# antoineleeman/robust-nonlinear-mpc

Hardware: AMD Instinct MI355X
Metric: QP solves/sec (whole node), rockETH N=20 batch=4096 closed-loop RTI MPC step from script x0 (higher is better)
Workload: dtype f64

## Files before the change

robust-nonlinear-mpc_amd/csrc/dynamics.hpp:

```cpp
#pragma once
#include <math.h>
#ifndef __HIPCC__
#ifndef __host__
#define __host__
#endif
#ifndef __device__
#define __device__
#endif
#endif
#define DYN_HD __host__ __device__ inline

namespace dyn {

struct Dual {
    double v, d;
    DYN_HD Dual() : v(0.0), d(0.0) {}
    DYN_HD Dual(double a) : v(a), d(0.0) {}
    DYN_HD Dual(double a, double b) : v(a), d(b) {}
};
DYN_HD Dual operator+(Dual a, Dual b) { return Dual(a.v + b.v, a.d + b.d); }
DYN_HD Dual operator-(Dual a, Dual b) { return Dual(a.v - b.v, a.d - b.d); }
DYN_HD Dual operator-(Dual a) { return Dual(-a.v, -a.d); }
DYN_HD Dual operator*(Dual a, Dual b) { return Dual(a.v * b.v, a.d * b.v + a.v * b.d); }
DYN_HD Dual operator/(Dual a, Dual b) { const double q = a.v / b.v; return Dual(q, (a.d - q * b.d) / b.v); }
DYN_HD Dual msin(Dual a) { return Dual(sin(a.v), cos(a.v) * a.d); }
DYN_HD Dual mcos(Dual a) { return Dual(cos(a.v), -sin(a.v) * a.d); }
DYN_HD Dual msqrt(Dual a) { const double s = sqrt(a.v); return Dual(s, 0.5 * a.d / s); }
DYN_HD Dual matan(Dual a) { return Dual(atan(a.v), a.d / (1.0 + a.v * a.v)); }
DYN_HD void msincos(double a, double &s, double &c) {
#ifdef __HIP_DEVICE_COMPILE__
    sincos(a, &s, &c);
#else
    s = sin(a); c = cos(a);
#endif
}
DYN_HD void msincos(Dual a, Dual &s, Dual &c) {
    double sv, cv;
    msincos(a.v, sv, cv);
    s = Dual(sv, cv * a.d); c = Dual(cv, -sv * a.d);
}
DYN_HD double msin(double a) { return sin(a); }
DYN_HD double mcos(double a) { return cos(a); }
DYN_HD double msqrt(double a) { return sqrt(a); }
// ... 148 lines not shown
    constexpr int NX = Dims<MODEL>::NX, NT = Dims<MODEL>::NT;
    const double h = RK4_H;
    double k[NX], t[NX], acc[NX];
    { MathRecord mf(tape); ode<MODEL, double, MathRecord>(x, u, k, mf); }
    for (int i = 0; i < NX; i++) { acc[i] = k[i]; t[i] = x[i] + 0.5 * h * k[i]; stage[i] = t[i]; }
    { MathRecord mf(tape + NT); ode<MODEL, double, MathRecord>(t, u, k, mf); }
    for (int i = 0; i < NX; i++) { acc[i] = acc[i] + 2.0 * k[i]; t[i] = x[i] + 0.5 * h * k[i]; stage[NX + i] = t[i]; }
    { MathRecord mf(tape + 2 * NT); ode<MODEL, double, MathRecord>(t, u, k, mf); }
    for (int i = 0; i < NX; i++) { acc[i] = acc[i] + 2.0 * k[i]; t[i] = x[i] + h * k[i]; stage[2 * NX + i] = t[i]; }
    { MathRecord mf(tape + 3 * NT); ode<MODEL, double, MathRecord>(t, u, k, mf); }
    for (int i = 0; i < NX; i++) xp[i] = x[i] + (1.0 / 6.0) * (acc[i] + k[i]) * h;
}
template <int MODEL>
DYN_HD void ddyn_tangent(const double *x, const double *u, const double *stage, const double *tape, int dir, double *col) {
    constexpr int NX = Dims<MODEL>::NX, NU = Dims<MODEL>::NU, NT = Dims<MODEL>::NT;
    const double h = RK4_H;
    Dual T[NX], U[NU], K[NX];
    double acc[NX];
    for (int i = 0; i < NU; i++) U[i] = Dual(u[i], NX + i == dir ? 1.0 : 0.0);
    for (int i = 0; i < NX; i++) { T[i] = Dual(x[i], i == dir ? 1.0 : 0.0); acc[i] = 0.0; }
#pragma unroll
    for (int s = 0; s < 4; s++) {
        { MathReplay mf(tape + s * NT); ode<MODEL, Dual, MathReplay>(T, U, K, mf); }
        const double w = (s == 0 || s == 3) ? 1.0 : 2.0, cn = (s == 2) ? h : 0.5 * h;
        for (int i = 0; i < NX; i++) {
            acc[i] += w * K[i].d;
            if (s < 3) T[i] = Dual(stage[s * NX + i], (i == dir ? 1.0 : 0.0) + cn * K[i].d);
        }
    }
    for (int i = 0; i < NX; i++) col[i] = (i == dir ? 1.0 : 0.0) + (h / 6.0) * acc[i];
}

}
```

robust-nonlinear-mpc_amd/csrc/slsqp_api.hip:

```cpp
#include <hip/hip_runtime.h>

#include <algorithm>
#include <cmath>
#include <cstdio>
#include <cstring>
#include <cstdlib>
#include <map>
#include <string>
#include <vector>

#include "../../include/slsqp.h"
#include "slsqp_kernels.hpp"

using namespace slsqp;

static thread_local std::string g_err;
static int fail(const std::string &m) { g_err = m; return -1; }
#define HIPCHK(x)                                                                                  \
    do {                                                                                           \
        hipError_t e_ = (x);                                                                       \
        if (e_ != hipSuccess) return fail(std::string(#x) + ": " + hipGetErrorString(e_));         \
    } while (0)

extern "C" const char *slsqp_last_error(void) { return g_err.c_str(); }
extern "C" const char *slsqp_version(void) { return "slsqp-hip 0.1 (gfx950)"; }

extern "C" void slsqp_default_opts(slsqp_opts *o) {
    o->rti_steps = 1; o->max_sls_iter = 30; o->qp_max_iter = 60; o->qp_eps = 1e-6; o->conv_tol = 1e-3;
    o->eps_backoff = 1e-10; o->want_K = 1; o->warm_start = 1; o->warm_rounds = 20;
    o->max_scp_iter = 100; o->scp_eps = 1e-10; o->precision = 0; o->time_kernels = 0; o->as_first = 2; o->as_rounds = 24; o->as_max_viol = 64; o->ipm_restart = 1; o->as_warm_max_set = 28; o->as_warm_last = 1; o->fuse_rti = 1; o->cl_persistent = 1;
}

struct slsqp_handle {
    slsqp_dims d;
    int B, dev, n, m, mb, nz;
    hipStream_t st;
    double *A, *Bm, *E, *g, *gN, *c, *q, *x0val, *gf_raw, *g_raw, *cst;
    int model_id;
    double *Xn, *Un, *xmeas, *x0arg, *u0, *wbuf, *u_init; int cl_steps;
    double *ubg, *lbg;
    double *primal, *dual, *cost, *pin_dual, *kkt, *prev_primal, *Linv, *ws, *qpstate;
    double *eta, *eta_f, *beta, *beta_f, *backoff, *backoff_f, *backoff_x, *backoff_u, *K;
    int *status, *iters, *itnum, *has_prev, *conv, *alive, *mask, *success, *infeas, *counter;
    int *scp_active, *scp_success, *scp_iters, *pending_reset, *scp_upd; double *scp_dmax;
    int horizon_shifted = 0;
    std::vector<hipEvent_t> tl; std::vector<int> tl_role; int tl_n = 0; double tl_acc[5] = {0, 0, 0, 0, 0};
    int *cl_stepno = nullptr, *cl_lag = nullptr, *cl_begin = nullptr, *cl_runm = nullptr, *cl_done = nullptr, *cl_skipb = nullptr, *cl_skip_begin = nullptr, *qplog = nullptr;
    double *call_ids = nullptr, *cl_W = nullptr; size_t cl_W_doubles = 0; unsigned long long *t0word = nullptr; int qplog_steps = 0, qplog_cap = 0, *qplog_nsolves = nullptr;
    int *clq_slots = nullptr, *clq_ctl = nullptr; unsigned clq_cap = 0; int cl_loop_waves = 0; double cl_loop_ms = 0.0; unsigned long long *cl_busy = nullptr, *cl_tbegin = nullptr, cl_busy_host[16] = {};
    bool cl_round = false; unsigned long long cl_budget = 0; int cl_total_steps = 0; unsigned cl_cut_count = 0xFFFFFFFFu;
    unsigned long long *chain_times = nullptr, *chain_times_host = nullptr;
    int *qp_diag = nullptr;
    double *nom_st; int *nom_need_lin, *nom_status, *nom_iters;
    int *retry; int mx_retry, mx_retry_total;
    int *databad, *runq;
    double *Kc, *Aclc;
    double *lin_stage, *lin_tape;
    double call_id;
    int *qpstat;
    double *x0viol;
    double x0_box_tol = 0.0;
    double x0_tol_dev = 0.0;
    double *x0vlog = nullptr;
    double *lg_x0v = nullptr;
    int *stale;
    double *pinf; double t_jac;
    int *mapA, *mapB;
    double *stage;
    size_t stage_bytes;
    bool have_costs, have_cons, have_dyn;
    bool beta_inited;
    bool general_G;
    double *Gd, *Gfd;
    hipEvent_t ev[10];
    std::vector<hipEvent_t> kev;
    int n_kev; bool time_kernels;
    double t_total, t_qp, t_sweep, t_fwd; int n_fwd; double fwd_inst;
    std::map<std::string, std::pair<void *, size_t>> named;
    unsigned long long *inst_launches;
    double *ct_part, *cost_tube;
    std::vector<void *> owned, log_owned;
    int log_steps;
    double *lg_x, *lg_u, *lg_bx, *lg_bu, *lg_state, *lg_u0, *lg_pinf; int *lg_succ, *lg_it;
};

static Costs costs_of(slsqp_handle *h) {
    const int nx = h->d.nx, nu = h->d.nu;
    Costs c;
    c.Qd = h->cst; c.Rd = c.Qd + nx; c.Qfd = c.Rd + nu; c.Qregd = c.Qfd + nx; c.Rregd = c.Qregd + nx; c.Qregfd = c.Rregd + nu; c.prox = 0.0;
    return c;
// ... 43 lines not shown
    if (d->N < 1 || d->N > 64 || batch < 1) { fail("need 1 <= N <= 64 and batch >= 1"); return nullptr; }
    int ndev = 0;
    if (hipGetDeviceCount(&ndev) != hipSuccess || ndev == 0) { fail("no HIP device visible: libslsqp_hip has no CPU fallback"); return nullptr; }
    if (hipSetDevice(device) != hipSuccess) { fail("hipSetDevice failed"); return nullptr; }
    slsqp_handle *h = new slsqp_handle();
    h->d = *d; h->B = batch; h->dev = device;
    const int nx = d->nx, nu = d->nu, N = d->N, ni = d->ni, nif = d->ni_f, nw = d->nw;
    h->nz = nx + nu; h->n = h->nz * N + nx; h->mb = N * (nx + ni) + nif; h->m = h->mb + nx;
    const size_t B = batch;
    if (hipStreamCreate(&h->st) != hipSuccess) { fail("hipStreamCreate"); delete h; return nullptr; }
    int rc = 0;
    rc |= dalloc(h->owned, &h->A, B * N * nx * nx); rc |= dalloc(h->owned, &h->Bm, B * N * nx * nu); rc |= dalloc(h->owned, &h->E, (size_t)(N + 1) * nx * nx);
    (void)nw;
    rc |= dalloc(h->owned, &h->g, B * N * ni); rc |= dalloc(h->owned, &h->gN, B * nif); rc |= dalloc(h->owned, &h->c, B * N * nx); rc |= dalloc(h->owned, &h->q, B * h->n);
    rc |= dalloc(h->owned, &h->x0val, B * nx); rc |= dalloc(h->owned, &h->gf_raw, (size_t)nif); rc |= dalloc(h->owned, &h->g_raw, (size_t)ni);
    rc |= dalloc(h->owned, &h->Xn, B * (N + 1) * nx); rc |= dalloc(h->owned, &h->Un, B * N * nu); rc |= dalloc(h->owned, &h->xmeas, B * nx); rc |= dalloc(h->owned, &h->x0arg, B * nx);
    rc |= dalloc(h->owned, &h->u0, B * nu); rc |= dalloc(h->owned, &h->wbuf, B * nx); rc |= dalloc(h->owned, &h->u_init, (size_t)nu); h->cl_steps = 0; rc |= dalloc(h->owned, &h->cst, (size_t)(3 * nx + 2 * nu) * 2);
    rc |= dalloc(h->owned, &h->ubg, B * h->mb); rc |= dalloc(h->owned, &h->lbg, B * h->mb);
    rc |= dalloc(h->owned, &h->primal, B * h->n); rc |= dalloc(h->owned, &h->dual, B * h->mb); rc |= dalloc(h->owned, &h->cost, B); rc |= dalloc(h->owned, &h->pin_dual, B * nx);
    rc |= dalloc(h->owned, &h->kkt, kkt_doubles(B)); rc |= dalloc(h->owned, &h->prev_primal, B * h->n); rc |= dalloc(h->owned, &h->Linv, B * N * nx * nx); rc |= dalloc(h->owned, &h->ws, B * qp_ws_doubles(h->n, N, nx)); rc |= dalloc(h->owned, &h->qpstate, B * 40);
    rc |= dalloc(h->owned, &h->eta, B * N * N * ni); rc |= dalloc(h->owned, &h->eta_f, B * (N + 1) * nif); rc |= dalloc(h->owned, &h->beta, B * N * N * ni);
    rc |= dalloc(h->owned, &h->beta_f, B * (N + 1) * nif); rc |= dalloc(h->owned, &h->backoff, B * N * ni); rc |= dalloc(h->owned, &h->backoff_f, B * nif);
    rc |= dalloc(h->owned, &h->backoff_x, B * (N + 1) * nx); rc |= dalloc(h->owned, &h->backoff_u, B * N * nu); rc |= dalloc(h->owned, &h->K, B * N * (N + 1) * nu * nx);
    rc |= dalloc(h->owned, &h->status, B); rc |= dalloc(h->owned, &h->iters, B); rc |= dalloc(h->owned, &h->itnum, B); rc |= dalloc(h->owned, &h->has_prev, B); rc |= dalloc(h->owned, &h->conv, B);
    rc |= dalloc(h->owned, &h->alive, B); rc |= dalloc(h->owned, &h->mask, B); rc |= dalloc(h->owned, &h->success, B); rc |= dalloc(h->owned, &h->infeas, B); rc |= dalloc(h->owned, &h->counter, (size_t)4);
    rc |= dalloc(h->owned, &h->scp_active, B); rc |= dalloc(h->owned, &h->scp_success, B); rc |= dalloc(h->owned, &h->scp_iters, B); rc |= dalloc(h->owned, &h->pending_reset, B); rc |= dalloc(h->owned, &h->scp_dmax, B);
    rc |= dalloc(h->owned, &h->retry, B); h->mx_retry = 0; h->mx_retry_total = 0; rc |= dalloc(h->owned, &h->databad, B); rc |= dalloc(h->owned, &h->runq, B);
    rc |= dalloc(h->owned, &h->nom_st, B * 12); rc |= dalloc(h->owned, &h->nom_need_lin, B); rc |= dalloc(h->owned, &h->nom_status, B); rc |= dalloc(h->owned, &h->nom_iters, B);
    rc |= dalloc(h->owned, &h->mapA, (size_t)N * nx * nx); rc |= dalloc(h->owned, &h->mapB, (size_t)N * nx * nu);
    rc |= dalloc(h->owned, &h->inst_launches, (size_t)8); rc |= dalloc(h->owned, &h->chain_times, B * 4);
    rc |= dalloc(h->owned, &h->cl_stepno, B); rc |= dalloc(h->owned, &h->cl_lag, B); rc |= dalloc(h->owned, &h->cl_begin, B); rc |= dalloc(h->owned, &h->cl_runm, B); rc |= dalloc(h->owned, &h->cl_done, B);
    { unsigned cap = 1; while (cap < 4u * (unsigned)B) cap <<= 1; h->clq_cap = cap; rc |= dalloc(h->owned, &h->clq_slots, (size_t)cap); rc |= dalloc(h->owned, &h->clq_ctl, (size_t)8); rc |= dalloc(h->owned, &h->cl_busy, (size_t)16); rc |= dalloc(h->owned, &h->cl_tbegin, (size_t)B); }
    rc |= dalloc(h->owned, &h->cl_skipb, B); rc |= dalloc(h->owned, &h->call_ids, B); rc |= dalloc(h->owned, &h->t0word, (size_t)2); rc |= dalloc(h->owned, &h->ct_part, B * (N + 1)); rc |= dalloc(h->owned, &h->cost_tube, B);
    rc |= dalloc(h->owned, &h->lin_stage, B * N * 3 * nx); rc |= dalloc(h->owned, &h->lin_tape, B * N * 4 * dyn::NT_MAX); rc |= dalloc(h->owned, &h->Kc, B * N * nu * nx); rc |= dalloc(h->owned, &h->Aclc, B * N * nx * nx); rc |= dalloc(h->owned, &h->qpstat, B * 16); rc |= dalloc(h->owned, &h->Gd, (size_t)ni * (nx + nu)); rc |= dalloc(h->owned, &h->Gfd, (size_t)nif * nx); h->general_G = false; h->beta_inited = false; rc |= dalloc(h->owned, &h->stale, B); rc |= dalloc(h->owned, &h->pinf, B); rc |= dalloc(h->owned, &h->scp_upd, B); h->t_jac = 0;
    h->log_steps = 0; h->lg_x = h->lg_u = h->lg_bx = h->lg_bu = h->lg_state = h->lg_u0 = h->lg_pinf = nullptr; h->lg_succ = h->lg_it = nullptr;
    if (rc) { free_all(h->owned); hipStreamDestroy(h->st); delete h; return nullptr; }
    if (hipHostMalloc((void **)&h->chain_times_host, 4 * sizeof(unsigned long long)) != hipSuccess) h->chain_times_host = nullptr;
    else memset(h->chain_times_host, 0, 4 * sizeof(unsigned long long));
    for (auto &e : h->ev) hipEventCreate(&e);
    h->tl.resize(2 * 256); for (auto &e : h->tl) hipEventCreate(&e);
    h->tl_role.assign(256, 0); h->tl_n = 0;
    h->kev.resize(2 * 256); for (auto &e : h->kev) hipEventCreate(&e);
    h->n_kev = 0; h->t_fwd = 0; h->n_fwd = 0; h->fwd_inst = 0; h->time_kernels = false; h->call_id = 0;
    {
        std::vector<int> mA((size_t)N * nx * nx), mB((size_t)N * nx * nu);
        int p = 0;
        for (int k = 0; k <= N; k++) {
            for (int j = 0; j < nx; j++) {
                if (k >= 1) p += 1;
                if (k < N) { for (int i = 0; i < nx; i++) mA[((size_t)k * nx + i) * nx + j] = p + i; p += nx; p += 2; }
                else p += 2;
                if (k == 0) p += 1;
            }
            if (k < N)
                for (int a = 0; a < nu; a++) {
                    for (int i = 0; i < nx; i++) mB[((size_t)k * nx + i) * nu + a] = p + i;
                    p += nx; p += 2;
                }
        }
        hipMemcpyAsync(h->mapA, mA.data(), mA.size() * sizeof(int), hipMemcpyHostToDevice, h->st);
        hipMemcpyAsync(h->mapB, mB.data(), mB.size() * sizeof(int), hipMemcpyHostToDevice, h->st);
        hipStreamSynchronize(h->st);
    }
    h->stage = nullptr; h->stage_bytes = 0;
    h->have_costs = h->have_cons = h->have_dyn = false; h->model_id = -1;
    h->t_total = h->t_qp = h->t_sweep = 0;
    auto reg = [&](const char *nm, void *p, size_t bytes) { h->named[nm] = {p, bytes}; };
// ... 432 lines not shown
    for (unsigned i = blockIdx.x * blockDim.x + threadIdx.x; i < cap; i += gridDim.x * blockDim.x) q.slots[i] = (i < (unsigned)B) ? (int)i + 1 : 0;
    if (blockIdx.x == 0 && threadIdx.x == 0) { *q.head = 0u; *q.tail = (unsigned)B; *q.avail = B; *q.err = 0; }
}
__device__ __forceinline__ void solve_begin_wave(const SolveBeginArgs &a, int b, int lane) {
    const int act = a.active ? a.active[b] : 1;
    if (a.x0 && lane < a.NX) a.x0val[(size_t)b * a.NX + lane] = -a.x0[(size_t)b * a.NX + lane];
    const int pend = a.pending[b];
    wla::wsync_mem();
    if (lane == 0) { a.alive[b] = act; a.infeas[b] = 0; a.success[b] = 0; }
    if (pend && act) {
        for (size_t o = lane; o < a.neta; o += 64) a.eta[(size_t)b * a.neta + o] = 0.0;
        for (size_t o = lane; o < a.netaf; o += 64) a.eta_f[(size_t)b * a.netaf + o] = 0.0;
        const int st = a.stale[b];
        wla::wsync_mem();
        if (lane == 0) { a.itnum[b] = 0; a.pending[b] = 0; a.stale[b] = st & ~16; }
    }
    const InitBackoffArgs &i = a.ib;
    if (i.run && !i.run[b]) return;
    const int NZ = i.NX + i.NU, NI = 2 * NZ, NIF = 2 * i.NX, N = i.N;
    const double sq = sqrt(i.eps);
    for (int o = lane; o < N * NI; o += 64) i.backoff[(size_t)b * N * NI + o] = N * sq;
    for (int o = lane; o < NIF; o += 64) i.backoff_f[(size_t)b * NIF + o] = (N + 1) * sq;
    for (int o = lane; o < (N + 1) * i.NX; o += 64) i.backoff_x[(size_t)b * (N + 1) * i.NX + o] = 0.0;
    for (int o = lane; o < N * i.NU; o += 64) i.backoff_u[(size_t)b * N * i.NU + o] = 0.0;
}
struct LoopArgs {
    ChainArgs c; ClArgs cl; LinArgs lin; BoundsArgs ba; SolveBeginArgs sb; ClLogArgs lg; ScpArgs sa;
    int steps, n, have_log, fence, keep_laggards;
    int *stepno; double *call_ids, *q; int *stale, *itnum, *pending, *scp_active;
    const double *W_all; double *pinf;
    ClQueue Q;
    unsigned long long *busy, *t_begin;
};
template <int MODEL>
__device__ CLW_FN void cl_step_begin(const LoopArgs &L, int b, int lane) {
    constexpr int NX = dyn::Dims<MODEL>::NX;
    const int s = L.stepno[b];
    if (lane == 0) L.t_begin[b] = wall_clock64();
#ifdef CL_LOOP_STAMP
    unsigned long long ts_ = wall_clock64();
#define CLSTAMP(i) do { wla::wsync_mem(); const unsigned long long t_ = wall_clock64(); if (lane == 0) atomicAdd(L.busy + (i), t_ - ts_); ts_ = t_; } while (0)
#else
#define CLSTAMP(i) do {} while (0)
#endif
    if (s > 0) {
        cl_shift_wave<MODEL>(L.cl, b, lane);
        for (int o = lane; o < L.n; o += 64) L.q[(size_t)b * L.n + o] = 0.0;
        const int st = L.stale[b];
        wla::wsync_mem();
        if (lane == 0) { L.stale[b] = (st & 8) | 3; L.itnum[b] = 0; L.pending[b] = 0; }
    }
    if (lane == 0) { L.call_ids[b] += 1.0; L.sa.scp_success[b] = 0; L.sa.scp_iters[b] = 0; }
    wla::wsync_mem();
    CLSTAMP(4);
    lin_wave<MODEL>(L.lin, L.ba, b, lane);
    CLSTAMP(5);
    if (lane < NX) L.cl.x0arg[(size_t)b * NX + lane] = L.cl.Xn[(size_t)b * (L.cl.N + 1) * NX + lane] - L.cl.xmeas[(size_t)b * NX + lane];
    wla::wsync_mem();
    solve_begin_wave(L.sb, b, lane);
    wla::wsync_mem();
    CLSTAMP(6);
}
template <int MODEL>
__device__ CLW_FN int cl_step_end(const LoopArgs &L, int b, int lane) {
    constexpr int NX = dyn::Dims<MODEL>::NX;
    const int s = L.stepno[b];
#ifdef CL_LOOP_STAMP
    unsigned long long ts_ = wall_clock64();
#endif
    if (lane == 0) L.scp_active[b] = 1;
    wla::wsync_mem();
    cl_scp_update_wave(L.cl, L.sa, b, lane);
    wla::wsync_mem();
    CLSTAMP(7);
    if (L.sa.updated[b]) cl_infeas_wave<MODEL>(L.cl, L.pinf, b, lane);
    wla::wsync_mem();
    CLSTAMP(8);
    if (L.have_log) {
        const int per = 2 * ((L.lg.N + 1) * L.lg.NX + L.lg.N * L.lg.NU);
        for (int o = lane; o < per; o += 64) cl_log_item(L.lg, b, o);
    }
    CLSTAMP(9);
    if (lane == 0) {
        cl_plant_one<MODEL>(L.cl, b, L.W_all ? L.W_all + (size_t)s * L.cl.B * NX : nullptr);
        L.stepno[b] = s + 1;
        if (L.busy) { atomicAdd(L.busy, wall_clock64() - L.t_begin[b]); atomicAdd(L.busy + 2, 1ULL); }
    }
    wla::wsync_mem();
    CLSTAMP(10);
    return (s + 1 < L.steps) ? s + 1 : 0;
}
template <int MODEL>
__global__ __launch_bounds__(64, QP_PERSIST_WAVES_PER_SIMD) void k_cl_loop(LoopArgs L) {
    constexpr int NX = dyn::Dims<MODEL>::NX, NU = dyn::Dims<MODEL>::NU;
    int lane = threadIdx.x;
    extern __shared__ double sm[];
    int b = -1;
#ifdef CL_LOOP_STAMP
    const unsigned long long tw0_ = wall_clock64();
    if (lane == 0) atomicMin(L.busy + 14, tw0_);
#endif
#pragma unroll 1
    for (;;) {
        asm volatile("" : "+v"(lane));
        if (b < 0) {
#ifdef CL_LOOP_STAMP
            const unsigned long long tp_ = wall_clock64();
#endif
            b = clq_pop(L.Q, lane);
            if (b < 0) break;
            if (L.fence & 1) __threadfence();
#ifdef CL_LOOP_STAMP
            if (lane == 0) atomicAdd(L.busy + 11, wall_clock64() - tp_);
#endif
        }
        cl_step_begin<MODEL>(L, b, lane);
        b = __builtin_amdgcn_readfirstlane(b);
        asm volatile("" : "+v"(lane));
        rti_chain_dev<NX, NU>(L.c, b, lane, sm);
        wla::wsync_mem();
        asm volatile("" : "+v"(lane));
        const int next = __builtin_amdgcn_readfirstlane(cl_step_end<MODEL>(L, b, lane));
        b = __builtin_amdgcn_readfirstlane(b);
        if (!next) { b = -1; continue; }
        const unsigned long long done_steps = __hip_atomic_load(L.busy + 2, __ATOMIC_RELAXED, __HIP_MEMORY_SCOPE_AGENT);
        const int behind = __builtin_amdgcn_readfirstlane(((unsigned long long)next * (unsigned long long)L.cl.B < done_steps) ? 1 : 0);
        if (behind && L.keep_laggards) continue;
#ifdef CL_LOOP_STAMP
        const unsigned long long tq_ = wall_clock64();
#endif
        if (L.fence & 2) __threadfence();
        clq_push(L.Q, b, lane);
        b = -1;
#ifdef CL_LOOP_STAMP
        if (lane == 0) atomicAdd(L.busy + 12, wall_clock64() - tq_);
#endif
    }
#ifdef CL_LOOP_STAMP
    if (lane == 0) { const unsigned long long te_ = wall_clock64(); atomicAdd(L.busy + 13, te_ - tw0_); atomicMax(L.busy + 15, te_); atomicAdd(L.busy + 1, 1ULL); }
#endif
}

struct ScpLoopArgs {
    LoopArgs L;
    int max_it, converge, rti_steps;
    int *nsolves;
};
template <int MODEL>
__device__ CLW_FN void cl_scp_step_begin(const LoopArgs &L, int b, int lane) {
    const int s = L.stepno[b];
    if (lane == 0) L.t_begin[b] = wall_clock64();
    if (s > 0) {
        cl_shift_wave<MODEL>(L.cl, b, lane);
        for (int o = lane; o < L.n; o += 64) L.q[(size_t)b * L.n + o] = 0.0;
        const int st = L.stale[b];
// ... 840 lines not shown
                     h->pinf, h->lg_x, h->lg_u, h->lg_bx, h->lg_bu, h->lg_state, h->lg_u0, h->lg_pinf, h->lg_succ, h->lg_it};
        hipLaunchKernelGGL(k_cl_log, dim3(1024), dim3(256), 0, h->st, la);
        hipLaunchKernelGGL(k_cl_log_x0v, dim3((2 * h->B + 255) / 256), dim3(256), 0, h->st, h->B, h->log_steps, h->cl_steps, h->x0viol, h->qpstat, h->lg_x0v);
        h->named["log_x0_viol"] = {h->lg_x0v, sizeof(double) * 2 * (size_t)h->log_steps};
    }
    if (h->model_id == 0) hipLaunchKernelGGL((k_cl_shift_plant<0>), dim3(gb), dim3(64), 0, h->st, a, 0, 1);
    else if (h->model_id == 1) hipLaunchKernelGGL((k_cl_shift_plant<1>), dim3(gb), dim3(64), 0, h->st, a, 0, 1);
    else hipLaunchKernelGGL((k_cl_shift_plant<2>), dim3(gb), dim3(64), 0, h->st, a, 0, 1);
    HIPCHK(hipGetLastError());
    HIPCHK(hipStreamSynchronize(h->st));
    tl_take(h);
    h->cl_steps++;
    return 0;
}

__global__ void k_cl_begin_flags(int B, const int *begin, int *scp_success, int *scp_iters) {
    const int b = blockIdx.x * blockDim.x + threadIdx.x;
    if (b < B && begin[b]) { scp_success[b] = 0; scp_iters[b] = 0; }
}
template <int MODEL>
static int launch_loop_t(slsqp_handle *h, LoopArgs &L, const ScpLoopArgs *S = nullptr) {
    constexpr int NX = dyn::Dims<MODEL>::NX, NU = dyn::Dims<MODEL>::NU;
    const size_t lds = sizeof(double) * std::max({(size_t)qp_lds_doubles<NX, NU>(h->d.N), (size_t)(2 * h->n + 8), (size_t)sweep_lds_doubles<NX, NU>(), (size_t)sweep_prop_lds_doubles<NX, NU>()});
    int cu = 0;
    if (hipDeviceGetAttribute(&cu, hipDeviceAttributeMultiprocessorCount, h->dev) != hipSuccess || cu <= 0) cu = 256;
    const int env_waves = getenv("SLSQP_LOOP_WAVES") ? atoi(getenv("SLSQP_LOOP_WAVES")) : 0;
    const int slots = env_waves > 0 ? env_waves : cu * 4 * QP_PERSIST_WAVES_PER_SIMD;
    const int grid = std::max(1, std::min(h->B, slots));
    h->cl_loop_waves = grid;
    const bool timed = h->time_kernels && h->n_kev + 2 <= (int)h->kev.size();
    if (timed) hipEventRecord(h->kev[h->n_kev], h->st);
    hipEventRecord(h->ev[8], h->st);
    if (S) hipLaunchKernelGGL((k_cl_loop_scp<MODEL>), dim3(grid), dim3(64), lds, h->st, *S);
    else hipLaunchKernelGGL((k_cl_loop<MODEL>), dim3(grid), dim3(64), lds, h->st, L);
    hipEventRecord(h->ev[9], h->st);
    if (timed) { hipEventRecord(h->kev[h->n_kev + 1], h->st); h->n_kev += 2; }
    HIPCHK(hipGetLastError());
    return 0;
}
static int cl_run_persistent(slsqp_handle *h, int steps, const double *dW, const slsqp_opts &o, int *rounds_out, bool scp = false, int scp_rti = 1) {
    const int max_it = !scp ? 1 : (scp_rti > 0 ? scp_rti : o.max_scp_iter);
    const slsqp_dims &d = h->d;
    const int B = h->B;
    if (!h->beta_inited) {
        hipLaunchKernelGGL(k_fill_doubles, dim3(1024), dim3(256), 0, h->st, h->beta, o.eps_backoff, (size_t)B * d.N * d.N * d.ni);
        hipLaunchKernelGGL(k_fill_doubles, dim3(1024), dim3(256), 0, h->st, h->beta_f, o.eps_backoff, (size_t)B * (d.N + 1) * d.ni_f);
        h->beta_inited = true;
    }
    h->time_kernels = o.time_kernels != 0;
    LoopArgs L;
    const int *active = scp ? h->scp_active : nullptr;
    L.c = make_chain_args(h, o, active, 1);
    L.c.q1.call_ids = L.c.q2.call_ids = h->call_ids;
    L.c.q1.shift_stepno = L.c.q2.shift_stepno = h->cl_stepno;
    L.c.qplog = h->qplog; L.c.x0vlog = h->x0vlog; L.c.stepno = h->cl_stepno; L.c.log_steps = h->qplog_steps;
    L.cl = cl_args(h, nullptr);
    L.lin = LinArgs{B, d.N, h->Xn, h->Un, h->g_raw, h->gf_raw, costs_of(h), h->A, h->Bm, h->c, h->g, h->gN, h->q, nullptr, h->lin_stage, h->lin_tape};
    L.ba = BoundsArgs{B, d.N, d.nx, d.ni, d.ni_f, h->g, h->gN, h->c, h->ubg, h->lbg, 1e-10, nullptr};
    L.sb = SolveBeginArgs{B, d.nx, h->x0arg, h->x0val, active, h->alive, h->infeas, h->success, h->pending_reset, h->itnum, h->stale,
                          h->eta, h->eta_f, (size_t)d.N * d.N * d.ni, (size_t)(d.N + 1) * d.ni_f,
                          InitBackoffArgs{B, d.N, d.nx, d.nu, o.eps_backoff, active, h->beta, h->beta_f, h->backoff, h->backoff_f, h->backoff_x, h->backoff_u, 0}, nullptr};
    L.lg = ClLogArgs{h->cl_stepno, nullptr, B, d.N, d.nx, d.nu, h->log_steps, 0, h->Xn, h->Un, h->backoff_x, h->backoff_u, h->scp_success, h->scp_iters,
                     h->pinf, h->lg_x, h->lg_u, h->lg_bx, h->lg_bu, h->lg_state, h->lg_u0, h->lg_pinf, h->lg_succ, h->lg_it};
    L.sa = ScpArgs{0, 0, o.scp_eps, h->scp_active, h->scp_success, h->scp_iters, h->counter + 2, h->scp_dmax, h->scp_upd};
    L.steps = steps; L.n = h->n; L.have_log = h->log_steps > 0 ? 1 : 0;
    L.keep_laggards = getenv("SLSQP_LOOP_KEEP") ? atoi(getenv("SLSQP_LOOP_KEEP")) : 1;
    L.fence = getenv("SLSQP_LOOP_FENCE") ? atoi(getenv("SLSQP_LOOP_FENCE")) : 3;
    L.stepno = h->cl_stepno; L.call_ids = h->call_ids; L.q = h->q; L.stale = h->stale; L.itnum = h->itnum; L.pending = h->pending_reset; L.scp_active = h->scp_active;
    L.W_all = dW; L.pinf = h->pinf;
    L.Q = ClQueue{h->clq_slots, h->clq_cap - 1u, (unsigned *)h->clq_ctl, (unsigned *)h->clq_ctl + 1, h->clq_ctl + 2, h->clq_ctl + 3};
    L.busy = h->cl_busy; L.t_begin = h->cl_tbegin;
    hipLaunchKernelGGL(k_clq_init, dim3(64), dim3(256), 0, h->st, B, L.Q);
    HIPCHK(hipMemsetAsync(h->cl_busy, 0, 16 * sizeof(unsigned long long), h->st));
    HIPCHK(hipMemsetAsync(h->cl_busy + 14, 0xFF, sizeof(unsigned long long), h->st));
    HIPCHK(hipMemsetAsync(h->counter + 2, 0, sizeof(int), h->st));
    const int tl_tot = tl_begin(h, 2), tl_c = tl_begin(h, 4);
    int rc = -1;
    ScpLoopArgs S{L, max_it, scp_rti <= 0 ? 1 : 0, o.rti_steps, h->qplog_nsolves};
    const ScpLoopArgs *Sp = scp ? &S : nullptr;
    if (h->model_id == 0) rc = launch_loop_t<0>(h, L, Sp);
    else if (h->model_id == 1) rc = launch_loop_t<1>(h, L, Sp);
    else rc = launch_loop_t<2>(h, L, Sp);
    if (rc) return -1;
    if (scp && S.converge) hipLaunchKernelGGL(k_cl_qplog_masked, dim3(steps), dim3(256), 0, h->st, B, steps, h->qplog_steps, h->qplog_nsolves, h->qplog, h->x0vlog);
    tl_end(h, tl_c); tl_end(h, tl_tot);
    int ctl[4] = {0, 0, 0, 0};
    std::vector<int> sn((size_t)B);
    HIPCHK(hipMemcpyAsync(ctl, h->clq_ctl, sizeof(ctl), hipMemcpyDeviceToHost, h->st));
    HIPCHK(hipMemcpyAsync(sn.data(), h->cl_stepno, sizeof(int) * (size_t)B, hipMemcpyDeviceToHost, h->st));
    HIPCHK(hipMemcpyAsync(h->cl_busy_host, h->cl_busy, 16 * sizeof(unsigned long long), hipMemcpyDeviceToHost, h->st));
    if (h->chain_times_host) {
        if (scp) memset(h->chain_times_host, 0, 4 * sizeof(unsigned long long));
        else HIPCHK(hipMemcpyAsync(h->chain_times_host, h->chain_times, 4 * sizeof(unsigned long long), hipMemcpyDeviceToHost, h->st));
    }
    HIPCHK(hipStreamSynchronize(h->st));
    tl_take(h);
    h->cl_loop_ms = ev_ms(h->ev[8], h->ev[9]);
    h->have_dyn = true;
    int unfinished = 0;
    for (int b = 0; b < B; b++) unfinished += sn[b] < steps ? 1 : 0;
    if (ctl[3] != 0 || unfinished != 0)
        return fail("slsqp_cl_run (persistent): the instance queue did not drain (err " + std::to_string(ctl[3]) + ", " + std::to_string(unfinished) + " instances short of their steps)");
    h->cl_steps = steps;
    h->call_id += (double)steps * max_it;
// ... 288 lines not shown
```

robust-nonlinear-mpc_amd/csrc/slsqp_kernels.hpp:

```cpp
#pragma once
#include <hip/hip_runtime.h>

#include "dynamics.hpp"
#include "wave_la.hpp"

namespace slsqp {

constexpr double BIGB = 1e19;
__device__ __forceinline__ double nan_max(double a, double b) { return fmax(a, b == b ? b : INFINITY); }
constexpr double EPS_PIN = 1e-10;
constexpr int ST_INIT = -1;

#ifndef NE_MFMA
#define NE_MFMA 1
#endif
#ifndef NE_GJ_MFMA
#define NE_GJ_MFMA 1
#endif

struct Costs {
    const double *Qd, *Rd, *Qfd;
    const double *Qregd, *Rregd, *Qregfd;
    double prox;
};
// ... 1873 lines not shown
    if (a.run && !a.run[b]) return;
    tighten_dev(a, b, threadIdx.x, blockDim.x);
}

struct InitBackoffArgs { int B, N, NX, NU; double eps; const int *run; double *beta, *beta_f, *backoff, *backoff_f, *backoff_x, *backoff_u; int fill_beta; };
__global__ void k_init_backoff(InitBackoffArgs a) {
    const int b = blockIdx.x;
    if (a.run && !a.run[b]) return;
    const int NZ = a.NX + a.NU, NI = 2 * NZ, NIF = 2 * a.NX, N = a.N;
    const double sq = sqrt(a.eps);
    if (a.fill_beta) {
        for (int o = threadIdx.x; o < N * N * NI; o += blockDim.x) a.beta[(size_t)b * N * N * NI + o] = a.eps;
        for (int o = threadIdx.x; o < (N + 1) * NIF; o += blockDim.x) a.beta_f[(size_t)b * (N + 1) * NIF + o] = a.eps;
    }
    for (int o = threadIdx.x; o < N * NI; o += blockDim.x) a.backoff[(size_t)b * N * NI + o] = N * sq;
    for (int o = threadIdx.x; o < NIF; o += blockDim.x) a.backoff_f[(size_t)b * NIF + o] = (N + 1) * sq;
    for (int o = threadIdx.x; o < (N + 1) * a.NX; o += blockDim.x) a.backoff_x[(size_t)b * (N + 1) * a.NX + o] = 0.0;
    for (int o = threadIdx.x; o < N * a.NU; o += blockDim.x) a.backoff_u[(size_t)b * N * a.NU + o] = 0.0;
}


struct LinArgs {
    int B, N;
    const double *X, *U, *g_raw, *gf_raw;
    Costs cst;
    double *A, *Bm, *c, *g, *gN, *q;
    const int *run;
    double *stage;
    double *tape;
};
#ifndef CLW_FN
#define CLW_FN __forceinline__
#endif
template <int MODEL>
__device__ __forceinline__ void lin_val_item(const LinArgs &a, int b, int k) {
    constexpr int NX = dyn::Dims<MODEL>::NX, NU = dyn::Dims<MODEL>::NU;
    const size_t t = (size_t)b * a.N + k;
    const double *xg = a.X + ((size_t)b * (a.N + 1) + k) * NX, *ug = a.U + ((size_t)b * a.N + k) * NU;
    double x[NX], u[NU], st[3 * NX], f[NX];
    for (int i = 0; i < NX; i++) x[i] = xg[i];
    for (int i = 0; i < NU; i++) u[i] = ug[i];
    dyn::ddyn_stages<MODEL>(x, u, st, f, a.tape + t * 4 * dyn::NT_MAX);
    double *sg = a.stage + t * 3 * NX, *c = a.c + t * NX;
    for (int i = 0; i < 3 * NX; i++) sg[i] = st[i];
    for (int i = 0; i < NX; i++) c[i] = f[i] - xg[NX + i];
}
template <int MODEL>
__global__ __launch_bounds__(128) void k_lin_val(LinArgs a) {
    const size_t tot = (size_t)a.B * a.N;
    for (size_t t = blockIdx.x * (size_t)blockDim.x + threadIdx.x; t < tot; t += (size_t)gridDim.x * blockDim.x) {
        const int k = t % a.N, b = t / a.N;
        if (a.run && !a.run[b]) continue;
        lin_val_item<MODEL>(a, b, k);
    }
}
template <int MODEL>
__device__ __forceinline__ void lin_tan_item(const LinArgs &a, int b, int k, int dir) {
    constexpr int NX = dyn::Dims<MODEL>::NX, NU = dyn::Dims<MODEL>::NU;
    const size_t bk = (size_t)b * a.N + k;
    const double *x = a.X + ((size_t)b * (a.N + 1) + k) * NX, *u = a.U + bk * NU;
    double col[NX];
    dyn::ddyn_tangent<MODEL>(x, u, a.stage + bk * 3 * NX, a.tape + bk * 4 * dyn::NT_MAX, dir, col);
    if (dir < NX) { double *A = a.A + bk * NX * NX; for (int i = 0; i < NX; i++) A[i * NX + dir] = col[i]; }
    else { double *Bm = a.Bm + bk * NX * NU; for (int i = 0; i < NX; i++) Bm[i * NU + (dir - NX)] = col[i]; }
}
template <int MODEL>
// ... 2 lines not shown
    const size_t tot = (size_t)a.B * a.N * NZ;
    for (size_t t = blockIdx.x * (size_t)blockDim.x + threadIdx.x; t < tot; t += (size_t)gridDim.x * blockDim.x) {
        const int dir = t % NZ, k = (t / NZ) % a.N, b = t / ((size_t)NZ * a.N);
        if (a.run && !a.run[b]) continue;
        lin_tan_item<MODEL>(a, b, k, dir);
    }
}
template <int NX, int NU>
__device__ __forceinline__ void lin_vec_item(const LinArgs &a, int b, int e) {
    constexpr int NZ = NX + NU, NI = 2 * NZ, NIF = 2 * NX;
    const int n = NZ * a.N + NX, k = e / NZ, i = e % NZ;
    const double z = (i < NX) ? a.X[((size_t)b * (a.N + 1) + k) * NX + i] : a.U[((size_t)b * a.N + k) * NU + (i - NX)];
    if (k < a.N) {
        double *g = a.g + ((size_t)b * a.N + k) * NI;
        g[i] = a.g_raw[i] - z; g[NZ + i] = a.g_raw[NZ + i] + z;
        a.q[(size_t)b * n + e] = 2.0 * (i < NX ? a.cst.Qd[i] : a.cst.Rd[i - NX]) * z;
    } else {
        double *g = a.gN + (size_t)b * NIF;
        g[i] = a.gf_raw[i] - z; g[NX + i] = a.gf_raw[NX + i] + z;
        a.q[(size_t)b * n + e] = 2.0 * a.cst.Qfd[i] * z;
    }
}
template <int NX, int NU>
__global__ void k_lin_vec(LinArgs a) {
    constexpr int NZ = NX + NU;
    const int n = NZ * a.N + NX;
    const size_t tot = (size_t)a.B * n;
    for (size_t t = blockIdx.x * (size_t)blockDim.x + threadIdx.x; t < tot; t += (size_t)gridDim.x * blockDim.x) {
        const int e = t % n, b = t / n;
        if (a.run && !a.run[b]) continue;
        lin_vec_item<NX, NU>(a, b, e);
    }
}
template <int MODEL>
__device__ CLW_FN void lin_wave(const LinArgs &a, const BoundsArgs &ba, int b, int lane) {
    constexpr int NX = dyn::Dims<MODEL>::NX, NU = dyn::Dims<MODEL>::NU, NZ = NX + NU;
    const int n = NZ * a.N + NX;
    if (lane < a.N) lin_val_item<MODEL>(a, b, lane);
    wla::wsync_mem();
    for (int t = lane; t < a.N * NZ; t += 64) lin_tan_item<MODEL>(a, b, t / NZ, t % NZ);
    for (int e = lane; e < n; e += 64) lin_vec_item<NX, NU>(a, b, e);
    wla::wsync_mem();
    const int mb = ba.N * (ba.NX + ba.NI) + ba.NIF;
    for (int r = lane; r < mb; r += 64) set_bounds_row(ba, b, r);
    wla::wsync_mem();
}


struct ClArgs {
    int B, N, NX, NU;
    double *Xn, *Un, *xmeas;
    const double *primal;
    const int *success;
    double *x0arg;
    const double *E, *w;
    double *u0;
    const double *u_init;
};
struct ScpArgs { int ii, converge; double eps; int *active, *scp_success, *scp_iters, *n_active; double *dmax; int *updated; };
__device__ __forceinline__ void cl_scp_update_wave(const ClArgs &a, const ScpArgs &s, int b, int lane) {
    if (!s.active[b]) { if (lane == 0) s.updated[b] = 0; return; }
    const int NZ = a.NX + a.NU, n = NZ * a.N + a.NX;
    if (!a.success[b]) {
        if (lane == 0) { s.active[b] = 0; s.scp_success[b] = 0; s.scp_iters[b] = s.ii; s.updated[b] = 0; }
        return;
    }
    const double *d = a.primal + (size_t)b * n;
    double dm = 0.0;
    for (int e = lane; e < n; e += 64) {
        const int k = e / NZ, i = e % NZ;
        const double dv = d[e];
// ... 92 lines not shown
        double s = xp[i];
        if (w) for (int j = 0; j < NX; j++) s += a.E[i * NX + j] * w[(size_t)b * NX + j];
        a.xmeas[(size_t)b * NX + i] = s;
    }
}
template <int MODEL>
__device__ __forceinline__ void cl_shift_tail(const ClArgs &a, int b, double *xp) {
    constexpr int NX = dyn::Dims<MODEL>::NX, NU = dyn::Dims<MODEL>::NU;
    const double *X = a.Xn + (size_t)b * (a.N + 1) * NX, *U = a.Un + (size_t)b * a.N * NU;
    double xN[NX], uN[NU];
    for (int i = 0; i < NX; i++) xN[i] = X[(size_t)a.N * NX + i];
    for (int i = 0; i < NU; i++) uN[i] = U[(size_t)(a.N - 1) * NU + i];
    dyn::ddyn<MODEL, double>(xN, uN, xp);
}
template <int MODEL>
__global__ void k_cl_shift_plant(ClArgs a, int do_shift, int do_plant, const int *mask = nullptr, const int *stepno = nullptr, const double *W_all = nullptr) {
    constexpr int NX = dyn::Dims<MODEL>::NX, NU = dyn::Dims<MODEL>::NU;
    const int b = blockIdx.x * blockDim.x + threadIdx.x;
    if (b >= a.B) return;
    if (mask && !mask[b]) return;
    if (do_shift && stepno && stepno[b] == 0) return;
    if (W_all) a.w = W_all + (size_t)stepno[b] * a.B * NX;
    double *X = a.Xn + (size_t)b * (a.N + 1) * NX, *U = a.Un + (size_t)b * a.N * NU;
    if (do_plant) cl_plant_one<MODEL>(a, b, a.w);
    if (do_shift) {
        double xp[NX];
        cl_shift_tail<MODEL>(a, b, xp);
        for (int k = 0; k < a.N; k++) for (int i = 0; i < NX; i++) X[(size_t)k * NX + i] = X[(size_t)(k + 1) * NX + i];
        for (int k = 0; k + 1 < a.N; k++) for (int i = 0; i < NU; i++) U[(size_t)k * NU + i] = U[(size_t)(k + 1) * NU + i];
        for (int i = 0; i < NX; i++) X[(size_t)a.N * NX + i] = xp[i];
    }
}
template <int MODEL>
__device__ CLW_FN void cl_shift_wave(const ClArgs &a, int b, int lane) {
    constexpr int NX = dyn::Dims<MODEL>::NX, NU = dyn::Dims<MODEL>::NU;
    double *X = a.Xn + (size_t)b * (a.N + 1) * NX, *U = a.Un + (size_t)b * a.N * NU;
    double xp[NX];
    if (lane == 0) cl_shift_tail<MODEL>(a, b, xp);
    constexpr int PX = (64 * NX + 63) / 64, PU = (63 * NU + 63) / 64;
    double vx[PX], vu[PU];
#pragma unroll
    for (int i = 0; i < PX; i++) { const int o = lane + 64 * i; vx[i] = (o < a.N * NX) ? X[o + NX] : 0.0; }
#pragma unroll
    for (int i = 0; i < PU; i++) { const int o = lane + 64 * i; vu[i] = (o < (a.N - 1) * NU) ? U[o + NU] : 0.0; }
    wla::wsync_mem();
#pragma unroll
    for (int i = 0; i < PX; i++) { const int o = lane + 64 * i; if (o < a.N * NX) X[o] = vx[i]; }
#pragma unroll
    for (int i = 0; i < PU; i++) { const int o = lane + 64 * i; if (o < (a.N - 1) * NU) U[o] = vu[i]; }
    if (lane == 0) for (int i = 0; i < NX; i++) X[(size_t)a.N * NX + i] = xp[i];
    wla::wsync_mem();
}
template <int MODEL>
__global__ void k_cl_rollout(ClArgs a) {
    constexpr int NX = dyn::Dims<MODEL>::NX, NU = dyn::Dims<MODEL>::NU;
    const int b = blockIdx.x * blockDim.x + threadIdx.x;
    if (b >= a.B) return;
    double *X = a.Xn + (size_t)b * (a.N + 1) * NX, *U = a.Un + (size_t)b * a.N * NU;
    double x[NX], u[NU], xp[NX];
    for (int i = 0; i < NX; i++) { x[i] = a.xmeas[(size_t)b * NX + i]; X[i] = x[i]; }
    for (int i = 0; i < NU; i++) u[i] = a.u_init[i];
    for (int k = 0; k < a.N; k++) {
        for (int i = 0; i < NU; i++) U[(size_t)k * NU + i] = u[i];
        dyn::ddyn<MODEL, double>(x, u, xp);
        for (int i = 0; i < NX; i++) { x[i] = xp[i]; X[(size_t)(k + 1) * NX + i] = xp[i]; }
    }
}

struct NomArgs {
    int B, N;
    double *Xn, *Un;
    const double *xmeas;
    const double *primal;
    const int *qp_status;
    const double *g_raw, *gf_raw;
    Costs cst;
    double *st;
    int *active, *need_lin, *status, *iters, *n_active;
    double rho, tol, w_max;
    int mode;
};
__device__ __forceinline__ double block_sum128(double v, double *red) {
    const int t = threadIdx.x;
// ... 125 lines not shown
```

Before: 1.575 million.

## Fuse infeasibility, plant step and next-step linearization into one dynamics pass

Adds a per-wave dynamics pass that evaluates the RK4 stages for every shooting node, the plant step and the shifted tail in a single loop. It stores the stage and tape data in the positions the next shifted step expects, so the next step's linearization can skip recomputing values, and it reuses the results for the infeasibility measure, the shift tail and the plant update. A priming pass and a readiness flag per instance are introduced, buffers grow to N+1 and N+2 nodes, and FP contraction is set explicitly in the dynamics header. The indexing of the shifted buffers is intricate, and the extra priming pass adds work on the first step.

```diff
diff --git a/robust-nonlinear-mpc_amd/csrc/dynamics.hpp b/robust-nonlinear-mpc_amd/csrc/dynamics.hpp
--- a/robust-nonlinear-mpc_amd/csrc/dynamics.hpp
+++ b/robust-nonlinear-mpc_amd/csrc/dynamics.hpp
@@ -9,6 +9,10 @@
 #endif
 #endif
 #define DYN_HD __host__ __device__ inline
+
+#ifdef __clang__
+#pragma clang fp contract(on)
+#endif
 
 namespace dyn {
 
@@ -223,3 +227,7 @@
 }
 
 }
+
+#ifdef __clang__
+#pragma clang fp contract(fast)
+#endif
diff --git a/robust-nonlinear-mpc_amd/csrc/slsqp_api.hip b/robust-nonlinear-mpc_amd/csrc/slsqp_api.hip
--- a/robust-nonlinear-mpc_amd/csrc/slsqp_api.hip
+++ b/robust-nonlinear-mpc_amd/csrc/slsqp_api.hip
@@ -56,6 +56,7 @@
     int *databad, *runq;
     double *Kc, *Aclc;
     double *lin_stage, *lin_tape;
+    double *cl_dyn_xp = nullptr; int *cl_lin_ready = nullptr;
     double call_id;
     int *qpstat;
     double *x0viol;
@@ -165,7 +166,7 @@
     rc |= dalloc(h->owned, &h->cl_stepno, B); rc |= dalloc(h->owned, &h->cl_lag, B); rc |= dalloc(h->owned, &h->cl_begin, B); rc |= dalloc(h->owned, &h->cl_runm, B); rc |= dalloc(h->owned, &h->cl_done, B);
     { unsigned cap = 1; while (cap < 4u * (unsigned)B) cap <<= 1; h->clq_cap = cap; rc |= dalloc(h->owned, &h->clq_slots, (size_t)cap); rc |= dalloc(h->owned, &h->clq_ctl, (size_t)8); rc |= dalloc(h->owned, &h->cl_busy, (size_t)16); rc |= dalloc(h->owned, &h->cl_tbegin, (size_t)B); }
     rc |= dalloc(h->owned, &h->cl_skipb, B); rc |= dalloc(h->owned, &h->call_ids, B); rc |= dalloc(h->owned, &h->t0word, (size_t)2); rc |= dalloc(h->owned, &h->ct_part, B * (N + 1)); rc |= dalloc(h->owned, &h->cost_tube, B);
-    rc |= dalloc(h->owned, &h->lin_stage, B * N * 3 * nx); rc |= dalloc(h->owned, &h->lin_tape, B * N * 4 * dyn::NT_MAX); rc |= dalloc(h->owned, &h->Kc, B * N * nu * nx); rc |= dalloc(h->owned, &h->Aclc, B * N * nx * nx); rc |= dalloc(h->owned, &h->qpstat, B * 16); rc |= dalloc(h->owned, &h->Gd, (size_t)ni * (nx + nu)); rc |= dalloc(h->owned, &h->Gfd, (size_t)nif * nx); h->general_G = false; h->beta_inited = false; rc |= dalloc(h->owned, &h->stale, B); rc |= dalloc(h->owned, &h->pinf, B); rc |= dalloc(h->owned, &h->scp_upd, B); h->t_jac = 0;
+    rc |= dalloc(h->owned, &h->lin_stage, B * (N + 1) * 3 * nx); rc |= dalloc(h->owned, &h->lin_tape, B * (N + 1) * 4 * dyn::NT_MAX); rc |= dalloc(h->owned, &h->cl_dyn_xp, B * (N + 2) * nx); rc |= dalloc(h->owned, &h->cl_lin_ready, B); rc |= dalloc(h->owned, &h->Kc, B * N * nu * nx); rc |= dalloc(h->owned, &h->Aclc, B * N * nx * nx); rc |= dalloc(h->owned, &h->qpstat, B * 16); rc |= dalloc(h->owned, &h->Gd, (size_t)ni * (nx + nu)); rc |= dalloc(h->owned, &h->Gfd, (size_t)nif * nx); h->general_G = false; h->beta_inited = false; rc |= dalloc(h->owned, &h->stale, B); rc |= dalloc(h->owned, &h->pinf, B); rc |= dalloc(h->owned, &h->scp_upd, B); h->t_jac = 0;
     h->log_steps = 0; h->lg_x = h->lg_u = h->lg_bx = h->lg_bu = h->lg_state = h->lg_u0 = h->lg_pinf = nullptr; h->lg_succ = h->lg_it = nullptr;
     if (rc) { free_all(h->owned); hipStreamDestroy(h->st); delete h; return nullptr; }
     if (hipHostMalloc((void **)&h->chain_times_host, 4 * sizeof(unsigned long long)) != hipSuccess) h->chain_times_host = nullptr;
@@ -664,11 +665,11 @@
     ClQueue Q;
     unsigned long long *busy, *t_begin;
 };
+struct LoopPassArgs { double *dyn_xp; int *lin_ready; };
 template <int MODEL>
-__device__ CLW_FN void cl_step_begin(const LoopArgs &L, int b, int lane) {
+__device__ CLW_FN void cl_step_begin(const LoopArgs &L, const LoopPassArgs &P, int b, int lane) {
     constexpr int NX = dyn::Dims<MODEL>::NX;
     const int s = L.stepno[b];
-    if (lane == 0) L.t_begin[b] = wall_clock64();
 #ifdef CL_LOOP_STAMP
     unsigned long long ts_ = wall_clock64();
 #define CLSTAMP(i) do { wla::wsync_mem(); const unsigned long long t_ = wall_clock64(); if (lane == 0) atomicAdd(L.busy + (i), t_ - ts_); ts_ = t_; } while (0)
@@ -676,16 +677,16 @@
 #define CLSTAMP(i) do {} while (0)
 #endif
     if (s > 0) {
-        cl_shift_wave<MODEL>(L.cl, b, lane);
+        cl_shift_wave<MODEL>(L.cl, b, lane, P.dyn_xp + ((size_t)b * (L.cl.N + 2) + L.cl.N) * NX);
         for (int o = lane; o < L.n; o += 64) L.q[(size_t)b * L.n + o] = 0.0;
         const int st = L.stale[b];
         wla::wsync_mem();
         if (lane == 0) { L.stale[b] = (st & 8) | 3; L.itnum[b] = 0; L.pending[b] = 0; }
     }
-    if (lane == 0) { L.call_ids[b] += 1.0; L.sa.scp_success[b] = 0; L.sa.scp_iters[b] = 0; }
+    if (lane == 0) { L.call_ids[b] += 1.0; L.sa.scp_success[b] = 0; L.sa.scp_iters[b] = 0; P.lin_ready[b] = 0; }
     wla::wsync_mem();
     CLSTAMP(4);
-    lin_wave<MODEL>(L.lin, L.ba, b, lane);
+    lin_wave<MODEL, true>(L.lin, L.ba, b, lane);
     CLSTAMP(5);
     if (lane < NX) L.cl.x0arg[(size_t)b * NX + lane] = L.cl.Xn[(size_t)b * (L.cl.N + 1) * NX + lane] - L.cl.xmeas[(size_t)b * NX + lane];
     wla::wsync_mem();
@@ -693,10 +694,7 @@
     wla::wsync_mem();
     CLSTAMP(6);
 }
-template <int MODEL>
-__device__ CLW_FN int cl_step_end(const LoopArgs &L, int b, int lane) {
-    constexpr int NX = dyn::Dims<MODEL>::NX;
-    const int s = L.stepno[b];
+__device__ CLW_FN void cl_step_update(const LoopArgs &L, int b, int lane) {
 #ifdef CL_LOOP_STAMP
     unsigned long long ts_ = wall_clock64();
 #endif
@@ -705,16 +703,18 @@
     cl_scp_update_wave(L.cl, L.sa, b, lane);
     wla::wsync_mem();
     CLSTAMP(7);
-    if (L.sa.updated[b]) cl_infeas_wave<MODEL>(L.cl, L.pinf, b, lane);
-    wla::wsync_mem();
-    CLSTAMP(8);
+}
+__device__ CLW_FN int cl_step_finish(const LoopArgs &L, int b, int lane) {
+    const int s = L.stepno[b];
+#ifdef CL_LOOP_STAMP
+    unsigned long long ts_ = wall_clock64();
+#endif
     if (L.have_log) {
         const int per = 2 * ((L.lg.N + 1) * L.lg.NX + L.lg.N * L.lg.NU);
         for (int o = lane; o < per; o += 64) cl_log_item(L.lg, b, o);
     }
     CLSTAMP(9);
     if (lane == 0) {
-        cl_plant_one<MODEL>(L.cl, b, L.W_all ? L.W_all + (size_t)s * L.cl.B * NX : nullptr);
         L.stepno[b] = s + 1;
         if (L.busy) { atomicAdd(L.busy, wall_clock64() - L.t_begin[b]); atomicAdd(L.busy + 2, 1ULL); }
     }
@@ -723,11 +723,11 @@
     return (s + 1 < L.steps) ? s + 1 : 0;
 }
 template <int MODEL>
-__global__ __launch_bounds__(64, QP_PERSIST_WAVES_PER_SIMD) void k_cl_loop(LoopArgs L) {
+__global__ __launch_bounds__(64, QP_PERSIST_WAVES_PER_SIMD) void k_cl_loop(LoopArgs L, LoopPassArgs P) {
     constexpr int NX = dyn::Dims<MODEL>::NX, NU = dyn::Dims<MODEL>::NU;
     int lane = threadIdx.x;
     extern __shared__ double sm[];
-    int b = -1;
+    int b = -1, primed = 0;
 #ifdef CL_LOOP_STAMP
     const unsigned long long tw0_ = wall_clock64();
     if (lane == 0) atomicMin(L.busy + 14, tw0_);
@@ -746,13 +746,35 @@
             if (lane == 0) atomicAdd(L.busy + 11, wall_clock64() - tp_);
 #endif
         }
-        cl_step_begin<MODEL>(L, b, lane);
+        const int s = __builtin_amdgcn_readfirstlane(L.stepno[b]);
+        const int prime = __builtin_amdgcn_readfirstlane(P.lin_ready[b]) ? 0 : 1;
+        if (!primed && lane == 0) L.t_begin[b] = wall_clock64();
+        if (!prime) {
+            cl_step_begin<MODEL>(L, P, b, lane);
+            b = __builtin_amdgcn_readfirstlane(b);
+            asm volatile("" : "+v"(lane));
+            rti_chain_dev<NX, NU>(L.c, b, lane, sm);
+            wla::wsync_mem();
+            asm volatile("" : "+v"(lane));
+            cl_step_update(L, b, lane);
+            b = __builtin_amdgcn_readfirstlane(b);
+        }
+        asm volatile("" : "+v"(lane));
+        {
+#ifdef CL_LOOP_STAMP
+            unsigned long long ts_ = wall_clock64();
+#endif
+            const int mode = prime ? (s > 0 ? CLP_PRIME : CLP_FIRST) : (s + 1 < L.steps ? CLP_STEP : CLP_LAST);
+            cl_dyn_pass_wave<MODEL>(L.cl, L.lin, P.dyn_xp + (size_t)b * (L.cl.N + 2) * NX, L.pinf, L.sa.updated[b], L.W_all ? L.W_all + (size_t)s * L.cl.B * NX : nullptr, b, lane, mode);
+            if (lane == 0) P.lin_ready[b] = mode != CLP_LAST;
+            wla::wsync_mem();
+            CLSTAMP(prime ? 5 : 8);
+        }
         b = __builtin_amdgcn_readfirstlane(b);
+        primed = prime;
+        if (prime) continue;
         asm volatile("" : "+v"(lane));
-        rti_chain_dev<NX, NU>(L.c, b, lane, sm);
-        wla::wsync_mem();
-        asm volatile("" : "+v"(lane));
-        const int next = __builtin_amdgcn_readfirstlane(cl_step_end<MODEL>(L, b, lane));
+        const int next = __builtin_amdgcn_readfirstlane(cl_step_finish(L, b, lane));
         b = __builtin_amdgcn_readfirstlane(b);
         if (!next) { b = -1; continue; }
         const unsigned long long done_steps = __hip_atomic_load(L.busy + 2, __ATOMIC_RELAXED, __HIP_MEMORY_SCOPE_AGENT);
@@ -1659,7 +1681,7 @@
     if (timed) hipEventRecord(h->kev[h->n_kev], h->st);
     hipEventRecord(h->ev[8], h->st);
     if (S) hipLaunchKernelGGL((k_cl_loop_scp<MODEL>), dim3(grid), dim3(64), lds, h->st, *S);
-    else hipLaunchKernelGGL((k_cl_loop<MODEL>), dim3(grid), dim3(64), lds, h->st, L);
+    else hipLaunchKernelGGL((k_cl_loop<MODEL>), dim3(grid), dim3(64), lds, h->st, L, LoopPassArgs{h->cl_dyn_xp, h->cl_lin_ready});
     hipEventRecord(h->ev[9], h->st);
     if (timed) { hipEventRecord(h->kev[h->n_kev + 1], h->st); h->n_kev += 2; }
     HIPCHK(hipGetLastError());
@@ -1697,6 +1719,7 @@
     L.W_all = dW; L.pinf = h->pinf;
     L.Q = ClQueue{h->clq_slots, h->clq_cap - 1u, (unsigned *)h->clq_ctl, (unsigned *)h->clq_ctl + 1, h->clq_ctl + 2, h->clq_ctl + 3};
     L.busy = h->cl_busy; L.t_begin = h->cl_tbegin;
+    HIPCHK(hipMemsetAsync(h->cl_lin_ready, 0, sizeof(int) * (size_t)B, h->st));
     hipLaunchKernelGGL(k_clq_init, dim3(64), dim3(256), 0, h->st, B, L.Q);
     HIPCHK(hipMemsetAsync(h->cl_busy, 0, 16 * sizeof(unsigned long long), h->st));
     HIPCHK(hipMemsetAsync(h->cl_busy + 14, 0xFF, sizeof(unsigned long long), h->st));
diff --git a/robust-nonlinear-mpc_amd/csrc/slsqp_kernels.hpp b/robust-nonlinear-mpc_amd/csrc/slsqp_kernels.hpp
--- a/robust-nonlinear-mpc_amd/csrc/slsqp_kernels.hpp
+++ b/robust-nonlinear-mpc_amd/csrc/slsqp_kernels.hpp
@@ -1929,6 +1929,18 @@
 #ifndef CLW_FN
 #define CLW_FN __forceinline__
 #endif
+#ifndef CL_DYN_FN
+#define CL_DYN_FN __forceinline__
+#endif
+template <int MODEL>
+__device__ CL_DYN_FN void dyn_stages_g(const double *xg, const double *ug, double *stage, double *tape, double *xp) {
+    constexpr int NX = dyn::Dims<MODEL>::NX, NU = dyn::Dims<MODEL>::NU;
+    double x[NX], u[NU], f[NX];
+    for (int i = 0; i < NX; i++) x[i] = xg[i];
+    for (int i = 0; i < NU; i++) u[i] = ug[i];
+    dyn::ddyn_stages<MODEL>(x, u, stage, f, tape);
+    for (int i = 0; i < NX; i++) xp[i] = f[i];
+}
 template <int MODEL>
 __device__ __forceinline__ void lin_val_item(const LinArgs &a, int b, int k) {
     constexpr int NX = dyn::Dims<MODEL>::NX, NU = dyn::Dims<MODEL>::NU;
@@ -1997,11 +2009,11 @@
         lin_vec_item<NX, NU>(a, b, e);
     }
 }
-template <int MODEL>
+template <int MODEL, bool have_val = false>
 __device__ CLW_FN void lin_wave(const LinArgs &a, const BoundsArgs &ba, int b, int lane) {
     constexpr int NX = dyn::Dims<MODEL>::NX, NU = dyn::Dims<MODEL>::NU, NZ = NX + NU;
     const int n = NZ * a.N + NX;
-    if (lane < a.N) lin_val_item<MODEL>(a, b, lane);
+    if (!have_val && lane < a.N) lin_val_item<MODEL>(a, b, lane);
     wla::wsync_mem();
     for (int t = lane; t < a.N * NZ; t += 64) lin_tan_item<MODEL>(a, b, t / NZ, t % NZ);
     for (int e = lane; e < n; e += 64) lin_vec_item<NX, NU>(a, b, e);
@@ -2160,11 +2172,14 @@
     }
 }
 template <int MODEL>
-__device__ CLW_FN void cl_shift_wave(const ClArgs &a, int b, int lane) {
+__device__ CLW_FN void cl_shift_wave(const ClArgs &a, int b, int lane, const double *tail = nullptr) {
     constexpr int NX = dyn::Dims<MODEL>::NX, NU = dyn::Dims<MODEL>::NU;
     double *X = a.Xn + (size_t)b * (a.N + 1) * NX, *U = a.Un + (size_t)b * a.N * NU;
     double xp[NX];
-    if (lane == 0) cl_shift_tail<MODEL>(a, b, xp);
+    if (lane == 0) {
+        if (tail) for (int i = 0; i < NX; i++) xp[i] = tail[i];
+        else cl_shift_tail<MODEL>(a, b, xp);
+    }
     constexpr int PX = (64 * NX + 63) / 64, PU = (63 * NU + 63) / 64;
     double vx[PX], vu[PU];
 #pragma unroll
@@ -2177,6 +2192,44 @@
 #pragma unroll
     for (int i = 0; i < PU; i++) { const int o = lane + 64 * i; if (o < (a.N - 1) * NU) U[o] = vu[i]; }
     if (lane == 0) for (int i = 0; i < NX; i++) X[(size_t)a.N * NX + i] = xp[i];
+    wla::wsync_mem();
+}
+enum { CLP_STEP = 0, CLP_LAST = 1, CLP_PRIME = 2, CLP_FIRST = 3 };
+template <int MODEL>
+__device__ CLW_FN void cl_dyn_pass_wave(const ClArgs &a, const LinArgs &lin, double *xpb, double *pinf, int updated, const double *w, int b, int lane, int mode) {
+    constexpr int NX = dyn::Dims<MODEL>::NX, NU = dyn::Dims<MODEL>::NU;
+    const int N = a.N;
+    const double *X = a.Xn + (size_t)b * (N + 1) * NX, *U = a.Un + (size_t)b * N * NU;
+    const int sh = mode == CLP_FIRST ? 0 : 1;
+    for (int k = lane; k < N + 2; k += 64) {
+        const double *xg = k <= N ? X + (size_t)k * NX : a.xmeas + (size_t)b * NX;
+        const double *ug = k < N ? U + (size_t)k * NU : k == N ? U + (size_t)(N - 1) * NU : U;
+        const bool keep = mode != CLP_LAST && k >= sh && k < N + sh;
+        const size_t slot = keep ? (size_t)b * N + (k - sh) : (size_t)lin.B * N + b;
+        dyn_stages_g<MODEL>(xg, ug, lin.stage + slot * 3 * NX, lin.tape + slot * 4 * dyn::NT_MAX, xpb + (size_t)k * NX);
+    }
+    wla::wsync_mem();
+    double mx = -1e300;
+    for (int k = lane; k <= N; k += 64) {
+        const double *xp = xpb + (size_t)k * NX, *xn = k < N ? X + (size_t)(k + 1) * NX : xp;
+        const bool keep = mode != CLP_LAST && k >= sh && k < N + sh;
+        double *c = lin.c + ((size_t)b * N + (k - sh)) * NX;
+        for (int i = 0; i < NX; i++) {
+            const double d = xp[i] - xn[i];
+            if (k < N) mx = fmax(mx, d);
+            if (keep) c[i] = d;
+        }
+    }
+    mx = wla::wave_max(mx);
+    if (mode <= CLP_LAST) {
+        if (updated && lane == 0) pinf[b] = mx;
+        if (lane < NU) a.u0[(size_t)b * NU + lane] = U[lane];
+        if (lane < NX) {
+            double s = xpb[(size_t)(N + 1) * NX + lane];
+            if (w) for (int j = 0; j < NX; j++) s += a.E[lane * NX + j] * w[(size_t)b * NX + j];
+            a.xmeas[(size_t)b * NX + lane] = s;
+        }
+    }
     wla::wsync_mem();
 }
 template <int MODEL>
```

After: 1.559 million. 0.99x the previous value.
